# stecrotti/MatrixProductBP.jl

Measured on AMD Instinct MI355X. Metric: edge-message updates/sec (and s/sweep), SIS 3-regular N=1024 T=50 d=20, higher is better.
Workload: dtype f64

## Files before the change

### matrixproductbp.jl_amd/csrc/wg_blocks.h

```cpp
#if !defined(WG_THREADS) || !defined(WG_WAVES)
#error "define WG_THREADS / WG_WAVES and include wg_common.h before wg_blocks.h (see kernels.h)"
#endif

namespace wg {

using namespace wgc;

constexpr int GM_MB = 96;
constexpr int GM_NT = 128;
constexpr int GM_KC = 32;
constexpr int GM_LDA = 112;
constexpr int GM_LDB = 144;
constexpr int GM_LDS_DOUBLES = GM_KC * (GM_LDA + GM_LDB);

template <bool NTX = false, bool NTO = false, class SP, class XP, class OP, class SRO, class SCO, class XRO, class XCO,
          class ORO, class OCO>
__device__ __attribute__((noinline)) void gemm_direct(int M, int N, int K, SP Sp, SRO sro, SCO sco,
                                                     XP Xp, XRO xro, XCO xco, OP Op, ORO oro, OCO oco,
                                                     bool accumulate, int tile0 = -1, int tstride = WG_WAVES);

template <class SRO, class SCO, class XRO, class XCO, class ORO, class OCO>
__device__ __attribute__((noinline)) void gemm(int M, int N, int K, const gdbl* Sp, SRO sro, SCO sco, const gdbl* Xp, XRO xro,
                     XCO xco, bool xkfast, gdbl* Op, ORO oro, OCO oco, bool accumulate, ldbl* lds) {
#if WG_THREADS != 512
// ... 526 lines not shown
    const int r = j0 + tid + WG_THREADS * s;
    rv[s] = r < rows;
#pragma unroll
    for (int c = 0; c < QR_NB; c++) P[s][c] = (rv[s] && c < nb) ? Y[(long)(j0 + c) * ld + r] : 0.0;
  }
  ldbl* tot = bc;
  ldbl* rowb = bc + 32;
  qr_panel_steps<0>(P, rv, Y, ld, j0, nb, red, tau, tot, rowb);
  __syncthreads();
}

template <bool TWO>
__device__ __forceinline__ void qr_gram(const gdbl* Y, long ld, int rows32, int jrow, int jx, int nbx, int jy,
                                        int nby, int jz, int nbz, ldbl* big) {
  const int tid = threadIdx.x, lane = tid & 63, wave = __builtin_amdgcn_readfirstlane(tid >> 6);
  const int g = lane >> 4, l15 = lane & 15;
  const int nrb = (rows32 - jrow) >> 4;
  const gdbl* xcol = Y + (long)(jx + l15) * ld + jrow + 4 * g;
  const gdbl* ycol = Y + (long)(jy + l15) * ld + jrow + 4 * g;
  const gdbl* zcol = Y + (long)(jz + l15) * ld + jrow + 4 * g;
  d4 acc1 = d4{0, 0, 0, 0}, acc2 = d4{0, 0, 0, 0};
  auto head = [&](d4& v, int rb, int jv, int nbv) {
#pragma unroll
    for (int e = 0; e < 4; e++) {
      const int rr = jrow + 16 * rb + 4 * g + e - jv;
      double a = v[e];
      a = (rr < 16) ? ((rr > l15) ? a : ((rr == l15) ? 1.0 : 0.0)) : a;
      v[e] = (l15 < nbv && rr >= 0 && rb < nrb) ? a : 0.0;
    }
  };
  d4 vx[2], vy[2], vz[2];
  auto load = [&](int rb, d4& a, d4& b, d4& c) {
    const int rbc = min(rb, nrb - 1);
    a = *reinterpret_cast<const gd4*>(xcol + 16 * rbc);
    b = *reinterpret_cast<const gd4*>(ycol + 16 * rbc);
    if (TWO) c = *reinterpret_cast<const gd4*>(zcol + 16 * rbc);
  };
  auto comp = [&](int rb, d4& a, d4& b, d4& c) {
    head(a, rb, jx, nbx); head(b, rb, jy, nby);
    if (TWO) head(c, rb, jz, nbz);
#pragma unroll
    for (int e = 0; e < 4; e++) {
      acc1 = mfma(a[e], b[e], acc1);
      if (TWO) acc2 = mfma(a[e], c[e], acc2);
    }
  };
  if (wave < nrb) load(wave, vx[0], vy[0], vz[0]);
  for (int rb = wave; rb < nrb; rb += 2 * WG_WAVES) {
    load(rb + WG_WAVES, vx[1], vy[1], vz[1]);
    comp(rb, vx[0], vy[0], vz[0]);
    load(rb + 2 * WG_WAVES, vx[0], vy[0], vz[0]);
    comp(rb + WG_WAVES, vx[1], vy[1], vz[1]);
  }
#pragma unroll
  for (int r = 0; r < 4; r++) {
    big[wave * 512 + (g + 4 * r) + 16 * l15] = acc1[r];
    if (TWO) big[wave * 512 + 256 + (g + 4 * r) + 16 * l15] = acc2[r];
  }
  __syncthreads();
  if (WG_WAVES > 1) {
    constexpr int NVAL = TWO ? 512 : 256;
    constexpr int PER = (NVAL + WG_THREADS - 1) / WG_THREADS;
    double s1[PER];
#pragma unroll
    for (int e = 0; e < PER; e++) {
      const int idx = tid + e * WG_THREADS;
      s1[e] = 0.0;
      if (idx < NVAL) {
#pragma unroll
        for (int w = 0; w < WG_WAVES; w++) s1[e] += big[w * 512 + idx];
      }
    }
    __syncthreads();
#pragma unroll
    for (int e = 0; e < PER; e++) {
      const int idx = tid + e * WG_THREADS;
      if (idx < NVAL) big[idx] = s1[e];
    }
    __syncthreads();
  }
}

template <int NP>
__device__ __forceinline__ void qr_gramN(const gdbl* Y, long ld, int rows32, int jrow, int jx, const int (&jy)[NP],
                                         ldbl* big) {
  const int tid = threadIdx.x, lane = tid & 63, wave = __builtin_amdgcn_readfirstlane(tid >> 6);
  const int g = lane >> 4, l15 = lane & 15;
  const int nrb = (rows32 - jrow) >> 4;
  const gdbl* xcol = Y + (long)(jx + l15) * ld + jrow + 4 * g;
  const gdbl* ycol[NP];
  d4 acc[NP];
#pragma unroll
  for (int k = 0; k < NP; k++) { ycol[k] = Y + (long)(jy[k] + l15) * ld + jrow + 4 * g; acc[k] = d4{0, 0, 0, 0}; }
  auto head = [&](d4& v, int rb, int jv) {
#pragma unroll
    for (int e = 0; e < 4; e++) {
      const int rr = jrow + 16 * rb + 4 * g + e - jv;
      double a = v[e];
      a = (rr < 16) ? ((rr > l15) ? a : ((rr == l15) ? 1.0 : 0.0)) : a;
      v[e] = (rr >= 0 && rb < nrb) ? a : 0.0;
    }
  };
  d4 vx[2], vy[2][NP];
  auto load = [&](int rb, d4& a, d4 (&b)[NP]) {
    const int rbc = min(rb, nrb - 1);
    a = *reinterpret_cast<const gd4*>(xcol + 16 * rbc);
#pragma unroll
    for (int k = 0; k < NP; k++) b[k] = *reinterpret_cast<const gd4*>(ycol[k] + 16 * rbc);
  };
  auto comp = [&](int rb, d4& a, d4 (&b)[NP]) {
    head(a, rb, jx);
#pragma unroll
    for (int k = 0; k < NP; k++) {
      head(b[k], rb, jy[k]);
#pragma unroll
      for (int e = 0; e < 4; e++) acc[k] = mfma(a[e], b[k][e], acc[k]);
    }
  };
  if (wave < nrb) load(wave, vx[0], vy[0]);
  for (int rb = wave; rb < nrb; rb += 2 * WG_WAVES) {
    load(rb + WG_WAVES, vx[1], vy[1]);
    comp(rb, vx[0], vy[0]);
    load(rb + 2 * WG_WAVES, vx[0], vy[0]);
    comp(rb + WG_WAVES, vx[1], vy[1]);
  }
  constexpr int NVAL = 256 * NP;
#pragma unroll
  for (int k = 0; k < NP; k++)
#pragma unroll
    for (int r = 0; r < 4; r++) big[wave * NVAL + 256 * k + (g + 4 * r) + 16 * l15] = acc[k][r];
  __syncthreads();
  if (WG_WAVES > 1) {
    constexpr int PER = (NVAL + WG_THREADS - 1) / WG_THREADS;
    double s1[PER];
#pragma unroll
    for (int e = 0; e < PER; e++) {
      const int idx = tid + e * WG_THREADS;
      s1[e] = 0.0;
      if (idx < NVAL) {
#pragma unroll
        for (int w2 = 0; w2 < WG_WAVES; w2++) s1[e] += big[w2 * NVAL + idx];
      }
    }
    __syncthreads();
#pragma unroll
    for (int e = 0; e < PER; e++) {
      const int idx = tid + e * WG_THREADS;
      if (idx < NVAL) big[idx] = s1[e];
    }
    __syncthreads();
  }
}

__device__ __forceinline__ void qr_T_from_gram(const ldbl* big, const ldbl* tau, int nb, ldbl* Ts) {
  const int tid = threadIdx.x;
  if (tid < 16) {
    double trow[16];
#pragma unroll
    for (int j = 0; j < 16; j++) {
      double gcol[16];
#pragma unroll
      for (int i2 = 0; i2 < 16; i2++) gcol[i2] = big[i2 + 16 * j];
      const double tj = tau[j];
      double sacc = 0.0;
#pragma unroll
      for (int i2 = 0; i2 < j; i2++) sacc += (i2 >= tid) ? trow[i2] * gcol[i2] : 0.0;
      double v = (j == tid) ? tj : ((j > tid) ? -tj * sacc : 0.0);
      trow[j] = (j < nb) ? v : 0.0;
    }
#pragma unroll
    for (int j = 0; j < 16; j++) Ts[tid + 16 * j] = trow[j];
  }
  __syncthreads();
}

__device__ __attribute__((noinline)) void qr_panel_global(gdbl* Y, long ld, int rows, int j0, int nb, ldbl* red, ldbl* Ts,
                                       ldbl* tau, ldbl* bc) {
  const int tid = threadIdx.x, lane = tid & 63, wave = __builtin_amdgcn_readfirstlane(tid >> 6);
  for (int jj = 0; jj < nb; jj++) {
    const int col = j0 + jj;
    gdbl* x = Y + (long)col * ld;
    double ss = 0.0;
    for (int r = col + 1 + tid; r < rows; r += WG_THREADS) { double v = x[r]; ss += v * v; }
    ss = wg_sum(ss, red);
    const double alpha = x[col];
    double beta, tj, scale;
    if (ss == 0.0) { beta = alpha; tj = 0.0; scale = 0.0; }
    else {
      beta = -copysign(sqrt(alpha * alpha + ss), alpha);
      tj = (beta - alpha) / beta;
      scale = 1.0 / (alpha - beta);
    }
    __syncthreads();
    for (int r = col + 1 + tid; r < rows; r += WG_THREADS) x[r] *= scale;
    if (tid == 0) { x[col] = beta; tau[jj] = tj; }
    __syncthreads();
    double part[QR_NB];
#pragma unroll
    for (int c = 0; c < QR_NB; c++) part[c] = 0.0;
    for (int r = col + 1 + tid; r < rows; r += WG_THREADS) {
      const double v = x[r];
#pragma unroll
      for (int c = 0; c < QR_NB; c++)
        if (c != jj && c < nb) part[c] += v * Y[(long)(j0 + c) * ld + r];
    }
#pragma unroll
    for (int c = 0; c < QR_NB; c++) part[c] = wave_sum(part[c]);
    if (lane == 0) {
#pragma unroll
      for (int c = 0; c < QR_NB; c++) red[wave * 16 + c] = part[c];
    }
    __syncthreads();
    if (tid < 16) {
      double s = 0.0;
#pragma unroll
      for (int w = 0; w < WG_WAVES; w++) s += red[w * 16 + tid];
      if (tid < nb && tid != jj) s += Y[(long)(j0 + tid) * ld + col];
      bc[tid] = s;
    }
    __syncthreads();
    for (int r = col + 1 + tid; r < rows; r += WG_THREADS) {
      const double v = x[r];
      for (int c = jj + 1; c < nb; c++) Y[(long)(j0 + c) * ld + r] -= tj * bc[c] * v;
    }
    if (tid > jj && tid < nb) Y[(long)(j0 + tid) * ld + col] -= tj * bc[tid];
    if (tid < jj) {
      double s = 0.0;
      for (int i2 = tid; i2 < jj; i2++) s += Ts[tid + 16 * i2] * bc[i2];
      Ts[tid + 16 * jj] = -tj * s;
    }
    if (tid == 0) Ts[jj + 16 * jj] = tj;
    __syncthreads();
  }
}

template <int NT>
__device__ __forceinline__ void qr_trail(gdbl* Y, long ld, int rows32, int j0, int nb, int cb0, const ldbl* Ts) {
  const int lane = threadIdx.x & 63;
  const int g = lane >> 4, l15 = lane & 15;
  const int nrb = (rows32 - j0) >> 4;
  const gdbl* vcol = Y + (long)(j0 + l15) * ld + j0 + 4 * g;
  const gdbl* ccol[NT];
  d4 w0[NT];
#pragma unroll
  for (int q = 0; q < NT; q++) { ccol[q] = Y + (long)(cb0 + 16 * q + l15) * ld + j0 + 4 * g; w0[q] = d4{0, 0, 0, 0}; }
  const bool vkeep = l15 < nb;
  {
    d4 sv[3], sc[3][NT];
    auto loadA = [&](int rb, d4& v, d4 (&c)[NT]) {
      const int rbc = min(rb, nrb - 1);
      v = *reinterpret_cast<const gd4*>(vcol + 16 * rbc);
#pragma unroll
      for (int q = 0; q < NT; q++) c[q] = *reinterpret_cast<const gd4*>(ccol[q] + 16 * rbc);
      const bool keep = vkeep && rb < nrb;
#pragma unroll
      for (int e = 0; e < 4; e++) {
        const int rho = 4 * g + e;
        double x = v[e];
        x = (rb == 0) ? ((rho > l15) ? x : ((rho == l15) ? 1.0 : 0.0)) : x;
        v[e] = keep ? x : 0.0;
      }
    };
    auto compA = [&](const d4& v, const d4 (&c)[NT]) {
#pragma unroll
      for (int e = 0; e < 4; e++)
#pragma unroll
        for (int q = 0; q < NT; q++) w0[q] = mfma(v[e], c[q][e], w0[q]);
    };
    loadA(0, sv[0], sc[0]);
    loadA(1, sv[1], sc[1]);
    for (int rb = 0; rb < nrb; rb += 3) {
      loadA(rb + 2, sv[2], sc[2]); compA(sv[0], sc[0]);
      loadA(rb + 3, sv[0], sc[0]); compA(sv[1], sc[1]);
      loadA(rb + 4, sv[1], sc[1]); compA(sv[2], sc[2]);
    }
  }
  d4 w[NT];
#pragma unroll
  for (int q = 0; q < NT; q++) {
    w[q] = d4{0, 0, 0, 0};
#pragma unroll
    for (int s = 0; s < 4; s++) w[q] = mfma(Ts[(4 * s + g) + 16 * l15], w0[q][s], w[q]);
  }
  {
    const int jb = j0 & ~31;
    const int nst = (rows32 - jb) >> 5;
    for (int st = 0; st < nst; st++) {
      const int row = jb + 32 * st + 2 * l15;
      d2 v[4];
#pragma unroll
      for (int s2 = 0; s2 < 4; s2++) {
        const int k = 4 * s2 + g;
        d2 x = *reinterpret_cast<const gd2*>(Y + (long)(j0 + k) * ld + row);
#pragma unroll
        for (int e = 0; e < 2; e++) {
          const int rho = row + e - j0;
          double xe = x[e];
          xe = (rho < 16) ? ((rho > k) ? xe : ((rho == k) ? 1.0 : 0.0)) : xe;
          x[e] = (k < nb && rho >= 0) ? xe : 0.0;
        }
        v[s2] = x;
      }
      d2 c[NT][4];
#pragma unroll
      for (int q = 0; q < NT; q++)
#pragma unroll
        for (int r = 0; r < 4; r++)
          c[q][r] = *reinterpret_cast<const gd2*>(Y + (long)(cb0 + 16 * q + g + 4 * r) * ld + row);
#pragma unroll
      for (int q = 0; q < NT; q++) {
#pragma unroll
        for (int e = 0; e < 2; e++) {
          d4 acc = d4{c[q][0][e], c[q][1][e], c[q][2][e], c[q][3][e]};
#pragma unroll
          for (int s2 = 0; s2 < 4; s2++) acc = mfma_na(w[q][s2], v[s2][e], acc);
#pragma unroll
          for (int r = 0; r < 4; r++) c[q][r][e] = acc[r];
        }
#pragma unroll
        for (int r = 0; r < 4; r++)
          *reinterpret_cast<gd2*>(Y + (long)(cb0 + 16 * q + g + 4 * r) * ld + row) = c[q][r];
      }
    }
  }
}

template <int NT>
__device__ __forceinline__ void qr_trail2(gdbl* Y, long ld, int rows32, int j0, int nbb, int cb0,
                                          const ldbl* TsA, const ldbl* TsB, const ldbl* Sm) {
  const int lane = threadIdx.x & 63;
  const int g = lane >> 4, l15 = lane & 15;
  const int nrb = (rows32 - j0) >> 4;
  const gdbl* vacol = Y + (long)(j0 + l15) * ld + j0 + 4 * g;
  const gdbl* vbcol = Y + (long)(j0 + 16 + l15) * ld + j0 + 4 * g;
  const gdbl* ccol[NT];
  d4 wa0[NT], wb0[NT];
#pragma unroll
  for (int q = 0; q < NT; q++) {
    ccol[q] = Y + (long)(cb0 + 16 * q + l15) * ld + j0 + 4 * g;
    wa0[q] = d4{0, 0, 0, 0}; wb0[q] = d4{0, 0, 0, 0};
  }
  const bool bkeep = l15 < nbb;
  {
    d4 sa[3], sb[3], sc[3][NT];
    auto loadA = [&](int rb, d4& va, d4& vb, d4 (&c)[NT]) {
      const int rbc = min(rb, nrb - 1);
      va = *reinterpret_cast<const gd4*>(vacol + 16 * rbc);
      vb = *reinterpret_cast<const gd4*>(vbcol + 16 * rbc);
#pragma unroll
      for (int q = 0; q < NT; q++) c[q] = *reinterpret_cast<const gd4*>(ccol[q] + 16 * rbc);
      const bool in = rb < nrb;
#pragma unroll
      for (int e = 0; e < 4; e++) {
        const int rho = 4 * g + e;
        double a = va[e], b = vb[e];
        a = (rb == 0) ? ((rho > l15) ? a : ((rho == l15) ? 1.0 : 0.0)) : a;
        b = (rb == 1) ? ((rho > l15) ? b : ((rho == l15) ? 1.0 : 0.0)) : b;
        va[e] = in ? a : 0.0;
        vb[e] = (in && bkeep && rb >= 1) ? b : 0.0;
      }
    };
    auto compA = [&](const d4& va, const d4& vb, const d4 (&c)[NT]) {
#pragma unroll
      for (int e = 0; e < 4; e++)
#pragma unroll
        for (int q = 0; q < NT; q++) { wa0[q] = mfma(va[e], c[q][e], wa0[q]); wb0[q] = mfma(vb[e], c[q][e], wb0[q]); }
    };
    loadA(0, sa[0], sb[0], sc[0]);
    loadA(1, sa[1], sb[1], sc[1]);
    for (int rb = 0; rb < nrb; rb += 3) {
      loadA(rb + 2, sa[2], sb[2], sc[2]); compA(sa[0], sb[0], sc[0]);
      loadA(rb + 3, sa[0], sb[0], sc[0]); compA(sa[1], sb[1], sc[1]);
      loadA(rb + 4, sa[1], sb[1], sc[1]); compA(sa[2], sb[2], sc[2]);
    }
  }
  d4 wa[NT], wb[NT];
#pragma unroll
  for (int q = 0; q < NT; q++) {
    wa[q] = d4{0, 0, 0, 0};
#pragma unroll
    for (int s = 0; s < 4; s++) wa[q] = mfma(TsA[(4 * s + g) + 16 * l15], wa0[q][s], wa[q]);
    d4 t = wb0[q];
#pragma unroll
    for (int s = 0; s < 4; s++) t = mfma_na(Sm[l15 + 16 * (4 * s + g)], wa[q][s], t);
    wb[q] = d4{0, 0, 0, 0};
#pragma unroll
    for (int s = 0; s < 4; s++) wb[q] = mfma(TsB[(4 * s + g) + 16 * l15], t[s], wb[q]);
  }
  {
    const int jb = j0 & ~31;
    const int nst = (rows32 - jb) >> 5;
    for (int st = 0; st < nst; st++) {
      const int row = jb + 32 * st + 2 * l15;
      d2 va[4], vb[4];
#pragma unroll
      for (int s2 = 0; s2 < 4; s2++) {
        const int k = 4 * s2 + g;
        d2 xa = *reinterpret_cast<const gd2*>(Y + (long)(j0 + k) * ld + row);
        d2 xb = *reinterpret_cast<const gd2*>(Y + (long)(j0 + 16 + k) * ld + row);
#pragma unroll
        for (int e = 0; e < 2; e++) {
          const int ra = row + e - j0, rbb = row + e - j0 - 16;
          double a = xa[e], b = xb[e];
          a = (ra < 16) ? ((ra > k) ? a : ((ra == k) ? 1.0 : 0.0)) : a;
          b = (rbb < 16) ? ((rbb > k) ? b : ((rbb == k) ? 1.0 : 0.0)) : b;
          xa[e] = (ra >= 0) ? a : 0.0;
          xb[e] = (k < nbb && rbb >= 0) ? b : 0.0;
        }
        va[s2] = xa; vb[s2] = xb;
      }
      d2 c[NT][4];
#pragma unroll
      for (int q = 0; q < NT; q++)
#pragma unroll
        for (int r = 0; r < 4; r++)
          c[q][r] = *reinterpret_cast<const gd2*>(Y + (long)(cb0 + 16 * q + g + 4 * r) * ld + row);
#pragma unroll
      for (int q = 0; q < NT; q++) {
#pragma unroll
        for (int e = 0; e < 2; e++) {
          d4 acc = d4{c[q][0][e], c[q][1][e], c[q][2][e], c[q][3][e]};
#pragma unroll
          for (int s2 = 0; s2 < 4; s2++) { acc = mfma_na(wa[q][s2], va[s2][e], acc); acc = mfma_na(wb[q][s2], vb[s2][e], acc); }
#pragma unroll
          for (int r = 0; r < 4; r++) c[q][r][e] = acc[r];
        }
#pragma unroll
        for (int r = 0; r < 4; r++)
          *reinterpret_cast<gd2*>(Y + (long)(cb0 + 16 * q + g + 4 * r) * ld + row) = c[q][r];
      }
    }
  }
}

__device__ __forceinline__ void qr_tile_update_all(gdbl* Y, long ld, int rows32, int j0, int nb, int cb0,
                                                   const ldbl* Ts, ldbl* big) {
  const int tid = threadIdx.x, lane = tid & 63, wave = __builtin_amdgcn_readfirstlane(tid >> 6);
  const int g = lane >> 4, l15 = lane & 15;
  const int nrb = (rows32 - j0) >> 4;
  const gdbl* vcol = Y + (long)(j0 + l15) * ld + j0 + 4 * g;
  const gdbl* ccol = Y + (long)(cb0 + l15) * ld + j0 + 4 * g;
  d4 acc = d4{0, 0, 0, 0};
  for (int rb = wave; rb < nrb; rb += WG_WAVES) {
    d4 v = *reinterpret_cast<const gd4*>(vcol + 16 * rb);
    d4 c = *reinterpret_cast<const gd4*>(ccol + 16 * rb);
#pragma unroll
    for (int e = 0; e < 4; e++) {
      const int rho = 4 * g + e;
      double x = v[e];
      x = (rb == 0) ? ((rho > l15) ? x : ((rho == l15) ? 1.0 : 0.0)) : x;
      v[e] = (l15 < nb) ? x : 0.0;
    }
#pragma unroll
    for (int e = 0; e < 4; e++) acc = mfma(v[e], c[e], acc);
  }
#pragma unroll
  for (int r = 0; r < 4; r++) big[wave * 256 + (g + 4 * r) + 16 * l15] = acc[r];
  __syncthreads();
  d4 w0 = d4{0, 0, 0, 0};
#pragma unroll
  for (int w = 0; w < WG_WAVES; w++)
#pragma unroll
    for (int r = 0; r < 4; r++) w0[r] += big[w * 256 + (g + 4 * r) + 16 * l15];
  d4 wv = d4{0, 0, 0, 0};
#pragma unroll
  for (int s = 0; s < 4; s++) wv = mfma(Ts[(4 * s + g) + 16 * l15], w0[s], wv);
  const int jb = j0 & ~31;
  const int nst = (rows32 - jb) >> 5;
  for (int st = wave; st < nst; st += WG_WAVES) {
    const int row = jb + 32 * st + 2 * l15;
    d2 v[4], c[4];
#pragma unroll
    for (int s2 = 0; s2 < 4; s2++) {
      const int k = 4 * s2 + g;
      d2 x = *reinterpret_cast<const gd2*>(Y + (long)(j0 + k) * ld + row);
#pragma unroll
      for (int e = 0; e < 2; e++) {
        const int rho = row + e - j0;
        double xe = x[e];
        xe = (rho < 16) ? ((rho > k) ? xe : ((rho == k) ? 1.0 : 0.0)) : xe;
        x[e] = (k < nb && rho >= 0) ? xe : 0.0;
      }
      v[s2] = x;
    }
#pragma unroll
    for (int r = 0; r < 4; r++) c[r] = *reinterpret_cast<const gd2*>(Y + (long)(cb0 + g + 4 * r) * ld + row);
#pragma unroll
    for (int e = 0; e < 2; e++) {
      d4 a = d4{c[0][e], c[1][e], c[2][e], c[3][e]};
#pragma unroll
      for (int s2 = 0; s2 < 4; s2++) a = mfma_na(wv[s2], v[s2][e], a);
#pragma unroll
      for (int r = 0; r < 4; r++) c[r][e] = a[r];
    }
#pragma unroll
    for (int r = 0; r < 4; r++) *reinterpret_cast<gd2*>(Y + (long)(cb0 + g + 4 * r) * ld + row) = c[r];
  }
  __syncthreads();
}

template <int NT>
__device__ __forceinline__ void qr_tile_update2_all(gdbl* Y, long ld, int rows32, int j0, int cb0, const ldbl* TsA,
                                                    const ldbl* TsB, const ldbl* Sm, ldbl* big) {
  const int tid = threadIdx.x, lane = tid & 63, wave = __builtin_amdgcn_readfirstlane(tid >> 6);
  const int g = lane >> 4, l15 = lane & 15;
  const int nrb = (rows32 - j0) >> 4;
  const gdbl* vacol = Y + (long)(j0 + l15) * ld + j0 + 4 * g;
  const gdbl* vbcol = Y + (long)(j0 + 16 + l15) * ld + j0 + 4 * g;
  d4 acca[NT], accb[NT];
#pragma unroll
  for (int q = 0; q < NT; q++) { acca[q] = d4{0, 0, 0, 0}; accb[q] = d4{0, 0, 0, 0}; }
  for (int rb = wave; rb < nrb; rb += WG_WAVES) {
    d4 va = *reinterpret_cast<const gd4*>(vacol + 16 * rb);
    d4 vb = *reinterpret_cast<const gd4*>(vbcol + 16 * rb);
    d4 c[NT];
#pragma unroll
    for (int q = 0; q < NT; q++) c[q] = *reinterpret_cast<const gd4*>(Y + (long)(cb0 + 16 * q + l15) * ld + j0 + 4 * g + 16 * rb);
#pragma unroll
    for (int e = 0; e < 4; e++) {
      const int rho = 4 * g + e;
      double a = va[e], b = vb[e];
      a = (rb == 0) ? ((rho > l15) ? a : ((rho == l15) ? 1.0 : 0.0)) : a;
      b = (rb == 1) ? ((rho > l15) ? b : ((rho == l15) ? 1.0 : 0.0)) : b;
      va[e] = a;
      vb[e] = (rb >= 1) ? b : 0.0;
    }
#pragma unroll
    for (int e = 0; e < 4; e++)
#pragma unroll
      for (int q = 0; q < NT; q++) { acca[q] = mfma(va[e], c[q][e], acca[q]); accb[q] = mfma(vb[e], c[q][e], accb[q]); }
  }
  constexpr int NVAL = 512 * NT;
#pragma unroll
  for (int q = 0; q < NT; q++)
#pragma unroll
    for (int r = 0; r < 4; r++) {
      big[wave * NVAL + 512 * q + (g + 4 * r) + 16 * l15] = acca[q][r];
      big[wave * NVAL + 512 * q + 256 + (g + 4 * r) + 16 * l15] = accb[q][r];
    }
  __syncthreads();
  d4 wa[NT], wb[NT];
#pragma unroll
  for (int q = 0; q < NT; q++) {
    d4 wa0 = d4{0, 0, 0, 0}, wb0 = d4{0, 0, 0, 0};
#pragma unroll
    for (int w = 0; w < WG_WAVES; w++)
#pragma unroll
      for (int r = 0; r < 4; r++) {
        wa0[r] += big[w * NVAL + 512 * q + (g + 4 * r) + 16 * l15];
        wb0[r] += big[w * NVAL + 512 * q + 256 + (g + 4 * r) + 16 * l15];
      }
    wa[q] = d4{0, 0, 0, 0}; wb[q] = d4{0, 0, 0, 0};
#pragma unroll
    for (int s = 0; s < 4; s++) wa[q] = mfma(TsA[(4 * s + g) + 16 * l15], wa0[s], wa[q]);
    d4 t = wb0;
#pragma unroll
    for (int s = 0; s < 4; s++) t = mfma_na(Sm[l15 + 16 * (4 * s + g)], wa[q][s], t);
#pragma unroll
    for (int s = 0; s < 4; s++) wb[q] = mfma(TsB[(4 * s + g) + 16 * l15], t[s], wb[q]);
  }
  const int jb = j0 & ~31;
  const int nst = (rows32 - jb) >> 5;
  for (int st = wave; st < nst; st += WG_WAVES) {
    const int row = jb + 32 * st + 2 * l15;
    d2 va[4], vb[4];
#pragma unroll
    for (int s2 = 0; s2 < 4; s2++) {
      const int k = 4 * s2 + g;
      d2 xa = *reinterpret_cast<const gd2*>(Y + (long)(j0 + k) * ld + row);
      d2 xb = *reinterpret_cast<const gd2*>(Y + (long)(j0 + 16 + k) * ld + row);
#pragma unroll
      for (int e = 0; e < 2; e++) {
        const int ra = row + e - j0, rbb = row + e - j0 - 16;
        double a = xa[e], b = xb[e];
        a = (ra < 16) ? ((ra > k) ? a : ((ra == k) ? 1.0 : 0.0)) : a;
        b = (rbb < 16) ? ((rbb > k) ? b : ((rbb == k) ? 1.0 : 0.0)) : b;
        xa[e] = (ra >= 0) ? a : 0.0;
        xb[e] = (rbb >= 0) ? b : 0.0;
      }
      va[s2] = xa; vb[s2] = xb;
    }
#pragma unroll
    for (int q = 0; q < NT; q++) {
      d2 c[4];
#pragma unroll
      for (int r = 0; r < 4; r++) c[r] = *reinterpret_cast<const gd2*>(Y + (long)(cb0 + 16 * q + g + 4 * r) * ld + row);
#pragma unroll
      for (int e = 0; e < 2; e++) {
        d4 acc = d4{c[0][e], c[1][e], c[2][e], c[3][e]};
#pragma unroll
        for (int s2 = 0; s2 < 4; s2++) { acc = mfma_na(wa[q][s2], va[s2][e], acc); acc = mfma_na(wb[q][s2], vb[s2][e], acc); }
#pragma unroll
        for (int r = 0; r < 4; r++) c[r][e] = acc[r];
      }
#pragma unroll
      for (int r = 0; r < 4; r++) *reinterpret_cast<gd2*>(Y + (long)(cb0 + 16 * q + g + 4 * r) * ld + row) = c[r];
    }
  }
  __syncthreads();
}

template <int NT>
__device__ __forceinline__ void qr_trail4(gdbl* Y, long ld, int rows32, int j0, int cb0, const ldbl* const (&Tq)[4],
                                          const ldbl* const (&Sq)[6]) {
  const int lane = threadIdx.x & 63;
  const int g = lane >> 4, l15 = lane & 15;
  const int nrb = (rows32 - j0) >> 4;
  const gdbl* vcol[4];
#pragma unroll
  for (int p = 0; p < 4; p++) vcol[p] = Y + (long)(j0 + 16 * p + l15) * ld + j0 + 4 * g;
  const gdbl* ccol[NT];
  d4 w0[4][NT];
#pragma unroll
  for (int q = 0; q < NT; q++) {
    ccol[q] = Y + (long)(cb0 + 16 * q + l15) * ld + j0 + 4 * g;
#pragma unroll
    for (int p = 0; p < 4; p++) w0[p][q] = d4{0, 0, 0, 0};
  }
  {
    d4 sv[2][4], sc[2][NT];
    auto loadA = [&](int rb, d4 (&v)[4], d4 (&c)[NT]) {
      const int rbc = min(rb, nrb - 1);
#pragma unroll
      for (int p = 0; p < 4; p++) v[p] = *reinterpret_cast<const gd4*>(vcol[p] + 16 * rbc);
#pragma unroll
      for (int q = 0; q < NT; q++) c[q] = __builtin_nontemporal_load(reinterpret_cast<const gd4*>(ccol[q] + 16 * rbc));
      const bool in = rb < nrb;
#pragma unroll
      for (int p = 0; p < 4; p++)
#pragma unroll
        for (int e = 0; e < 4; e++) {
          const int rho = 4 * g + e;
          double a = v[p][e];
          a = (rb == p) ? ((rho > l15) ? a : ((rho == l15) ? 1.0 : 0.0)) : a;
          v[p][e] = (in && rb >= p) ? a : 0.0;
        }
    };
    auto compA = [&](const d4 (&v)[4], const d4 (&c)[NT]) {
#pragma unroll
      for (int e = 0; e < 4; e++)
#pragma unroll
        for (int q = 0; q < NT; q++)
#pragma unroll
          for (int p = 0; p < 4; p++) w0[p][q] = mfma(v[p][e], c[q][e], w0[p][q]);
    };
    loadA(0, sv[0], sc[0]);
    for (int rb = 0; rb < nrb; rb += 2) {
      loadA(rb + 1, sv[1], sc[1]); compA(sv[0], sc[0]);
      loadA(rb + 2, sv[0], sc[0]); compA(sv[1], sc[1]);
    }
  }
  d4 w[4][NT];
#pragma unroll
  for (int q = 0; q < NT; q++) {
#pragma unroll
    for (int p = 0; p < 4; p++) {
      d4 t = w0[p][q];
#pragma unroll
      for (int r = 0; r < p; r++) {
        const ldbl* S = Sq[p * (p - 1) / 2 + r];
#pragma unroll
        for (int s = 0; s < 4; s++) t = mfma_na(S[l15 + 16 * (4 * s + g)], w[r][q][s], t);
      }
      d4 o = d4{0, 0, 0, 0};
#pragma unroll
      for (int s = 0; s < 4; s++) o = mfma(Tq[p][(4 * s + g) + 16 * l15], t[s], o);
      w[p][q] = o;
    }
  }
  {
    const int jb = j0 & ~31;
    const int nst = (rows32 - jb) >> 5;
    for (int st = 0; st < nst; st++) {
      const int row = jb + 32 * st + 2 * l15;
      d2 v[4][4];
#pragma unroll
      for (int p = 0; p < 4; p++)
#pragma unroll
        for (int s2 = 0; s2 < 4; s2++) {
          const int k = 4 * s2 + g;
          d2 x = *reinterpret_cast<const gd2*>(Y + (long)(j0 + 16 * p + k) * ld + row);
#pragma unroll
          for (int e = 0; e < 2; e++) {
            const int rp = row + e - j0 - 16 * p;
            double a = x[e];
            a = (rp < 16) ? ((rp > k) ? a : ((rp == k) ? 1.0 : 0.0)) : a;
            x[e] = (rp >= 0) ? a : 0.0;
          }
          v[p][s2] = x;
        }
      d2 c[NT][4];
#pragma unroll
      for (int q = 0; q < NT; q++)
#pragma unroll
        for (int r = 0; r < 4; r++)
          c[q][r] = __builtin_nontemporal_load(reinterpret_cast<const gd2*>(Y + (long)(cb0 + 16 * q + g + 4 * r) * ld + row));
#pragma unroll
      for (int q = 0; q < NT; q++) {
#pragma unroll
        for (int e = 0; e < 2; e++) {
          d4 acc = d4{c[q][0][e], c[q][1][e], c[q][2][e], c[q][3][e]};
#pragma unroll
          for (int s2 = 0; s2 < 4; s2++)
#pragma unroll
// ... 185 lines not shown
              const d2 va = *reinterpret_cast<const ld2*>(vp), vbb = *reinterpret_cast<const ld2*>(vp + 2);
              const double v4[4] = {va[0], va[1], vbb[0], vbb[1]};
#pragma unroll
              for (int e = 0; e < 4; e++)
#pragma unroll
                for (int q = 0; q < NR; q++) w0[p][q] = mfma(v4[e], cc[q][rb][e], w0[p][q]);
            }
          }
#pragma unroll
          for (int q = 0; q < NR; q++) { cc[q][0] = cn[q][0]; cc[q][1] = cn[q][1]; }
        }
        stage_store(m + 1, h, vn);
      }
    }
  }
  d4 w[4][NR];
  if (NTL > 0) {
#pragma unroll
    for (int q = 0; q < NR; q++) {
#pragma unroll
      for (int p = 0; p < 4; p++) {
        d4 t = w0[p][q];
#pragma unroll
        for (int r = 0; r < p; r++) {
          const ldbl* S = Sq[p * (p - 1) / 2 + r];
#pragma unroll
          for (int s = 0; s < 4; s++) t = mfma_na(S[l15 + 16 * (4 * s + g)], w[r][q][s], t);
        }
        d4 o = d4{0, 0, 0, 0};
#pragma unroll
        for (int s = 0; s < 4; s++) o = mfma(Tq[p][(4 * s + g) + 16 * l15], t[s], o);
        w[p][q] = o;
      }
    }
  }
  {
    {
      const d4 v0 = stage_load(0, 0), v1 = stage_load(0, 1);
      __syncthreads();
      stage_store(0, 0, v0); stage_store(0, 1, v1);
    }
    gdbl* cp[NR];
#pragma unroll
    for (int q = 0; q < NR; q++) cp[q] = Y + (long)(cq[q] + g) * ld + j0 + 2 * l15;
    d2 cc[NR][4];
    if (NTL > 0) {
#pragma unroll
      for (int q = 0; q < NR; q++)
#pragma unroll
        for (int r = 0; r < 4; r++) cc[q][r] = __builtin_nontemporal_load(reinterpret_cast<const gd2*>(cp[q] + (long)(4 * r) * ld));
    }
    for (int m = 0; m < nms; m++) {
#pragma unroll 1
      for (int h = 0; h < 2; h++) {
        const d4 vn = stage_load(m + 1, h);
        const int s = 2 * m + h;
        const int sn = min(s + 1, nst - 1);
        d2 cn[NR][4];
        if (NTL > 0) {
#pragma unroll
          for (int q = 0; q < NR; q++)
#pragma unroll
            for (int r = 0; r < 4; r++)
              cn[q][r] = __builtin_nontemporal_load(reinterpret_cast<const gd2*>(cp[q] + (long)(4 * r) * ld + 32 * sn));
        }
        if (h == 0) lds_barrier();
        if (NTL > 0) {
          if (s < nst) {
            const ldbl* vb = Vs + (m & 1) * QR_VM_STAGE + 32 * h;
            d4 acc[NR][2];
#pragma unroll
            for (int q = 0; q < NR; q++)
#pragma unroll
              for (int e = 0; e < 2; e++) acc[q][e] = d4{cc[q][0][e], cc[q][1][e], cc[q][2][e], cc[q][3][e]};
#pragma unroll
            for (int p = 0; p < 4; p++)
#pragma unroll
              for (int s2 = 0; s2 < 4; s2++) {
                const d2 v = *reinterpret_cast<const ld2*>(vb + (16 * p + 4 * s2 + g) * QR_VM_LD + 2 * l15);
#pragma unroll
                for (int e = 0; e < 2; e++)
#pragma unroll
                  for (int q = 0; q < NR; q++) acc[q][e] = mfma_na(w[p][q][s2], v[e], acc[q][e]);
              }
#pragma unroll
            for (int q = 0; q < NR; q++)
#pragma unroll
              for (int r = 0; r < 4; r++)
                __builtin_nontemporal_store(d2{acc[q][0][r], acc[q][1][r]}, reinterpret_cast<gd2*>(cp[q] + (long)(4 * r) * ld + 32 * s));
          }
#pragma unroll
          for (int q = 0; q < NR; q++)
#pragma unroll
            for (int r = 0; r < 4; r++) cc[q][r] = cn[q][r];
        }
        stage_store(m + 1, h, vn);
      }
    }
  }
}

__device__ __attribute__((noinline)) void qr_trail4_coop(gdbl* Y, long ld, int rows32, int j0, int cstart, int ntl,
                                                         const ldbl* const (&Tq)[4], const ldbl* const (&Sq)[6], ldbl* Vs) {
  const int wave = __builtin_amdgcn_readfirstlane(threadIdx.x >> 6);
  const int nst = (rows32 - j0) >> 5;
  const int tbase = ntl / WG_WAVES, trem = ntl % WG_WAVES;
  const int tcnt = tbase + (wave < trem ? 1 : 0);
  const int tstart = wave * tbase + min(wave, trem);
  const int npass = (tbase + (trem ? 1 : 0) + 1) >> 1;
  for (int pass = 0; pass < npass; pass++) {
    const int t0 = 2 * pass;
    const int nt = __builtin_amdgcn_readfirstlane(max(0, min(2, tcnt - t0)));
    const int cb0 = cstart + 16 * (tstart + t0);
    if (nt == 2) qr_trail4_coop_pass<2>(Y, ld, j0, nst, cb0, cb0 + 16, Tq, Sq, Vs);
    else if (nt == 1) qr_trail4_coop_pass<1>(Y, ld, j0, nst, cb0, cb0, Tq, Sq, Vs);
    else qr_trail4_coop_pass<0>(Y, ld, j0, nst, cstart, cstart, Tq, Sq, Vs);
  }
  __syncthreads();
}

__device__ __attribute__((noinline)) void qr_r(gdbl* Y, long ld, int rows, int cols, ldbl* lds, ldbl* big, Prof* pr = nullptr,
                     unsigned long long* plast = nullptr, int ph_panel = 0, int ph_trail = 0, bool force_generic = false) {
  const int tid = threadIdx.x, lane = tid & 63, wave = __builtin_amdgcn_readfirstlane(tid >> 6);
  const int g = lane >> 4, l15 = lane & 15;
  ldbl* red = lds;
  ldbl* Ts = lds + 2 * WG_WAVES * 16;
  ldbl* tau = Ts + 256;
  ldbl* bc = tau + 16;
  const int kmax = min(rows, cols);
  const bool fine = pr && ph_panel < 0;
  const int rows16 = (rows + 15) & ~15;
  const int rows32 = (rows + 31) & ~31;

  ldbl* TsB = lds + QR_LDS_BASE;
  ldbl* Sm = TsB + 256;
  ldbl* tauB = Sm + 256;
  ldbl* TsC = lds + QR_LDS_PAIR;
  ldbl* TsD = TsC + 256;
  ldbl* Sdc = TsD + 256;
  ldbl* Sca = Sdc + 256;
  ldbl* Scb = Sca + 256;
  ldbl* Sda = Scb + 256;
  ldbl* Sdb = Sda + 256;
  ldbl* tauC = Sdb + 256;
  ldbl* tauD = tauC + 16;

  auto factor_panel = [&](int jp, int nbp, ldbl* Tp, ldbl* taup) {
    for (int i = tid; i < 256; i += WG_THREADS) Tp[i] = 0.0;
    if (tid < 16) taup[tid] = 0.0;
    __syncthreads();
    qr_panel_regs(Y, ld, rows, jp, nbp, red, taup, bc);
    if (fine) prof_mark(pr, *plast, 14);
  };
  auto factor_pair = [&](int jp, ldbl* T1, ldbl* tau1, ldbl* T2, ldbl* tau2, ldbl* S21) {
    factor_panel(jp, 16, T1, tau1);
    qr_gram<false>(Y, ld, rows32, jp, jp, 16, jp, 16, jp, 16, big);
    if (fine) prof_mark(pr, *plast, 15);
    qr_T_from_gram(big, tau1, 16, T1);
    if (pr) prof_mark(pr, *plast, fine ? 16 : ph_panel);
    qr_tile_update_all(Y, ld, rows32, jp, 16, jp + 16, T1, big);
    if (pr) prof_mark(pr, *plast, fine ? 17 : ph_trail);
    factor_panel(jp + 16, 16, T2, tau2);
    qr_gram<true>(Y, ld, rows32, jp, jp + 16, 16, jp + 16, 16, jp, 16, big);
    for (int i = tid; i < 256; i += WG_THREADS) S21[i] = big[256 + i];
    if (fine) prof_mark(pr, *plast, 15);
    qr_T_from_gram(big, tau2, 16, T2);
    if (pr) prof_mark(pr, *plast, fine ? 16 : ph_panel);
  };
  auto factor_pair2 = [&](int ja) {
    const int jc = ja + 32, jd = ja + 48;
    factor_panel(jc, 16, TsC, tauC);
    { const int jy[3] = {jc, ja, ja + 16}; qr_gramN<3>(Y, ld, rows32, jc, jc, jy, big); }
    for (int i = tid; i < 256; i += WG_THREADS) { Sca[i] = big[256 + i]; Scb[i] = big[512 + i]; }
    if (fine) prof_mark(pr, *plast, 15);
    qr_T_from_gram(big, tauC, 16, TsC);
    if (pr) prof_mark(pr, *plast, fine ? 16 : ph_panel);
    qr_tile_update_all(Y, ld, rows32, jc, 16, jd, TsC, big);
    if (pr) prof_mark(pr, *plast, fine ? 17 : ph_trail);
    factor_panel(jd, 16, TsD, tauD);
    { const int jy[4] = {jd, jc, ja, ja + 16}; qr_gramN<4>(Y, ld, rows32, jd, jd, jy, big); }
    for (int i = tid; i < 256; i += WG_THREADS) { Sdc[i] = big[256 + i]; Sda[i] = big[512 + i]; Sdb[i] = big[768 + i]; }
    if (fine) prof_mark(pr, *plast, 15);
    qr_T_from_gram(big, tauD, 16, TsD);
    if (pr) prof_mark(pr, *plast, fine ? 16 : ph_panel);
  };
  auto wave_tiles = [&](int cstart, int& tstart, int& tcnt) {
    const int ntl = (cols - cstart + 15) / 16;
    const int tbase = ntl / WG_WAVES, trem = ntl % WG_WAVES;
    tcnt = tbase + (wave < trem ? 1 : 0);
    tstart = wave * tbase + min(wave, trem);
  };

  for (int j0 = 0; j0 < kmax;) {
    const int nb = min(QR_NB, kmax - j0);
    const bool fast = !force_generic && rows - j0 <= QR_RS * WG_THREADS;
    const bool quad = QR_QUAD && fast && j0 + 64 <= kmax && j0 + 64 < cols;
    const bool pair = !quad && fast && j0 + 32 <= kmax && j0 + 32 < cols;
    if (quad) {
      factor_pair(j0, Ts, tau, TsB, tauB, Sm);
      qr_tile_update2_all<2>(Y, ld, rows32, j0, j0 + 32, Ts, TsB, Sm, big);
      if (pr) prof_mark(pr, *plast, fine ? 17 : ph_trail);
      factor_pair2(j0);
      const ldbl* const Tq[4] = {Ts, TsB, TsC, TsD};
      const ldbl* const Sq[6] = {Sm, Sca, Scb, Sda, Sdb, Sdc};
      const int ntl4 = (cols - (j0 + 64) + 15) / 16;
      if (WG_WAVES > 1 && ntl4 <= QR_ROWPAR_TILES) {
        for (int tl = 0; tl < ntl4; tl++) qr_tile_update4_all(Y, ld, rows32, j0, j0 + 64 + 16 * tl, Tq, Sq, big);
      } else if (WG_WAVES == 8 && !QR_TRAIL_PER_WAVE) {
        const int rem = ((ntl4 & 3) == 1 && ntl4 > 4) ? 1 : 0;
        qr_trail4_coop(Y, ld, rows32, j0, j0 + 64, ntl4 - rem, Tq, Sq, big);
        if (rem) qr_tile_update4_all(Y, ld, rows32, j0, j0 + 64 + 16 * (ntl4 - 1), Tq, Sq, big);
      } else {
        int tstart, tcnt;
        wave_tiles(j0 + 64, tstart, tcnt);
        for (int tg = 0; tg < tcnt; tg += 2) {
          const int cb0 = j0 + 64 + (tstart + tg) * 16;
          if (tcnt - tg >= 2) qr_trail4<2>(Y, ld, rows32, j0, cb0, Tq, Sq);
          else qr_trail4<1>(Y, ld, rows32, j0, cb0, Tq, Sq);
        }
      }
      __syncthreads();
      if (pr) prof_mark(pr, *plast, fine ? 18 : ph_trail);
      j0 += 64;
      continue;
    }
    if (pair) factor_pair(j0, Ts, tau, TsB, tauB, Sm);
    else {
      for (int i = tid; i < 256; i += WG_THREADS) Ts[i] = 0.0;
      if (tid < 16) tau[tid] = 0.0;
      __syncthreads();
      if (fast) {
        qr_panel_regs(Y, ld, rows, j0, nb, red, tau, bc);
        if (fine) prof_mark(pr, *plast, 14);
        qr_gram<false>(Y, ld, rows32, j0, j0, nb, j0, nb, j0, nb, big);
        if (fine) prof_mark(pr, *plast, 15);
        qr_T_from_gram(big, tau, nb, Ts);
      } else qr_panel_global(Y, ld, rows, j0, nb, red, Ts, tau, bc);
      if (pr) prof_mark(pr, *plast, fine ? 16 : ph_panel);
    }
    const int cstart = pair ? j0 + 32 : j0 + nb;
    int tstart, tcnt;
    wave_tiles(cstart, tstart, tcnt);
    for (int tg = 0; tg < tcnt; tg += QR_TC) {
      const int nt = min(QR_TC, tcnt - tg);
      const int cb0 = cstart + (tstart + tg) * 16;
      if (pair) {
        if (nt == 1) qr_trail2<1>(Y, ld, rows32, j0, 16, cb0, Ts, TsB, Sm);
        else if (nt == 2) qr_trail2<2>(Y, ld, rows32, j0, 16, cb0, Ts, TsB, Sm);
        else qr_trail2<3>(Y, ld, rows32, j0, 16, cb0, Ts, TsB, Sm);
      } else {
        if (nt == 1) qr_trail<1>(Y, ld, rows32, j0, nb, cb0, Ts);
        else if (nt == 2) qr_trail<2>(Y, ld, rows32, j0, nb, cb0, Ts);
        else qr_trail<3>(Y, ld, rows32, j0, nb, cb0, Ts);
      }
    }
    __syncthreads();
    if (pr) prof_mark(pr, *plast, fine ? 18 : ph_trail);
    j0 += pair ? 32 : 16;
  }
  (void)g; (void)l15; (void)lane;
}

__device__ __forceinline__ void jac_cs(double al, double be, double ga, double& c, double& s) {
  const double d = be - al, g2 = 2.0 * ga;
  const double h2 = d * d + g2 * g2;
  double rs = __builtin_amdgcn_rsq(h2);
  rs = rs * (1.5 - 0.5 * h2 * rs * rs);
  double hy = h2 * rs;
  hy = hy + 0.5 * rs * (h2 - hy * hy);
  const double den = fabs(d) + hy;
  double rd = __builtin_amdgcn_rcp(den);
  rd = rd * (2.0 - den * rd);
  rd = rd * (2.0 - den * rd);
  const double t = copysign(g2, d * ga) * rd;
  const double o2 = 1.0 + t * t;
  c = __builtin_amdgcn_rsq(o2);
  c = c * (1.5 - 0.5 * o2 * c * c);
  c = c * (1.5 - 0.5 * o2 * c * c);
  s = c * t;
}

template <int R, class AP>
__device__ __forceinline__ double jac_pair8(AP ap, AP aq, int sub, double tol, double nul) {
  double x[R], y[R];
#pragma unroll
  for (int i = 0; i < R; i++) { x[i] = ap[sub + 8 * i]; y[i] = aq[sub + 8 * i]; }
  double al = 0, be = 0, ga = 0;
#pragma unroll
  for (int i = 0; i < R; i++) { al += x[i] * x[i]; be += y[i] * y[i]; ga += x[i] * y[i]; }
  al += dpp64<0x141>(al); be += dpp64<0x141>(be); ga += dpp64<0x141>(ga);
  al += dpp64<0x4E>(al); be += dpp64<0x4E>(be); ga += dpp64<0x4E>(ga);
  al += dpp64<0xB1>(al); be += dpp64<0xB1>(be); ga += dpp64<0xB1>(ga);
  if (!(ga * ga > (tol * tol) * (al * be) && al > nul && be > nul)) return 0.0;
  double c, s;
  jac_cs(al, be, ga, c, s);
#pragma unroll
  for (int i = 0; i < R; i++) { ap[sub + 8 * i] = c * x[i] - s * y[i]; aq[sub + 8 * i] = s * x[i] + c * y[i]; }
  return ga * ga / (al * be);
}

template <class T> struct jac_in_hbm { static constexpr bool value = false; };
template <> struct jac_in_hbm<gdbl*> { static constexpr bool value = true; };

__device__ __forceinline__ double jac_pair_hbm16(gdbl* ap, gdbl* aq, int sub, int m, double tol, double nul) {
  typedef double d2_t __attribute__((ext_vector_type(2)));
  typedef __attribute__((address_space(1))) d2_t gd2_t;
  constexpr int JP = 6;
  const int npl = (m + 15) >> 4;
  double al = 0, be = 0, ga = 0;
  d2_t x[JP], y[JP];
  auto loadc = [&](int j0) {
#pragma unroll
    for (int j = 0; j < JP; j++) {
      const int r = 2 * (sub + 8 * (j0 + j));
      const bool ok0 = r < m, ok1 = r + 1 < m;
      const int rc = ok1 ? r : 2 * sub;
      const d2_t xv = *reinterpret_cast<const gd2_t*>(ap + rc), yv = *reinterpret_cast<const gd2_t*>(aq + rc);
      x[j] = d2_t{ok0 && ok1 ? xv[0] : 0.0, ok1 ? xv[1] : 0.0};
      y[j] = d2_t{ok0 && ok1 ? yv[0] : 0.0, ok1 ? yv[1] : 0.0};
    }
  };
  for (int j0 = 0; j0 < npl; j0 += JP) {
    loadc(j0);
#pragma unroll
    for (int j = 0; j < JP; j++) {
      al += x[j][0] * x[j][0]; be += y[j][0] * y[j][0]; ga += x[j][0] * y[j][0];
      al += x[j][1] * x[j][1]; be += y[j][1] * y[j][1]; ga += x[j][1] * y[j][1];
    }
  }
  al += dpp64<0x141>(al); be += dpp64<0x141>(be); ga += dpp64<0x141>(ga);
  al += dpp64<0x4E>(al); be += dpp64<0x4E>(be); ga += dpp64<0x4E>(ga);
  al += dpp64<0xB1>(al); be += dpp64<0xB1>(be); ga += dpp64<0xB1>(ga);
  if (!(ga * ga > (tol * tol) * (al * be) && al > nul && be > nul)) return 0.0;
  double c, s;
  jac_cs(al, be, ga, c, s);
  for (int j0 = 0; j0 < npl; j0 += JP) {
    if (npl > JP) loadc(j0);
#pragma unroll
    for (int j = 0; j < JP; j++) {
      const int r = 2 * (sub + 8 * (j0 + j));
      if (r + 1 < m) {
        *reinterpret_cast<gd2_t*>(ap + r) = d2_t{c * x[j][0] - s * y[j][0], c * x[j][1] - s * y[j][1]};
        *reinterpret_cast<gd2_t*>(aq + r) = d2_t{s * x[j][0] + c * y[j][0], s * x[j][1] + c * y[j][1]};
      }
    }
  }
  return ga * ga / (al * be);
}

template <class AP>
__device__ __attribute__((noinline)) int jacobi_rsv(AP A, int lda, int m, int n, double* V, int ldv, ldbl* red,
                                                    __attribute__((address_space(3))) int* act, int maxsweeps) {
  const int tid = threadIdx.x;
  if (V) {
    for (int idx = tid; idx < n * n; idx += WG_THREADS) {
      int r = idx % n, c = idx / n;
      V[r + (long)ldv * c] = (r == c) ? 1.0 : 0.0;
    }
  }
  for (int c = tid; c < n; c += WG_THREADS) act[c] = c;
  __syncthreads();
  if (n < 2) return 0;
  double fro2 = 0.0;
  for (int idx = tid; idx < m * n; idx += WG_THREADS) { double v = A[(idx % m) + (long)lda * (idx / m)]; fro2 += v * v; }
  fro2 = wg_sum(fro2, red);
  const double nul = 1e-28 * fro2;
  const double tol = 1e-15;
  constexpr int JC = 12;
  int nact = n;
  int sweep = 0;
  bool conv = false;
  for (; sweep < maxsweeps; sweep++) {
    const int ne = (nact + 1) & ~1;
    const int npairs = ne / 2;
    int lg = 3;
    while (lg > 0 && (npairs << lg) > WG_THREADS) lg--;
    while (lg < 3 && ((m + (1 << lg) - 1) >> lg) > JC) lg++;
    const int LP = 1 << lg;
    const int sub = tid & (LP - 1);
// ... 106 lines not shown
```

Before: 547.8.

## Fuse QR trailing-update W0 products into multi-panel Gram reductions

```diff
diff --git a/matrixproductbp.jl_amd/csrc/wg_blocks.h b/matrixproductbp.jl_amd/csrc/wg_blocks.h
--- a/matrixproductbp.jl_amd/csrc/wg_blocks.h
+++ b/matrixproductbp.jl_amd/csrc/wg_blocks.h
@@ -702,6 +702,81 @@
   }
 }
 
+template <int NP, int NPR>
+__device__ __forceinline__ void qr_gram_multi(const gdbl* Y, long ld, int rows32, int jrow, const int (&jc)[NP],
+                                              const bool (&hd)[NP], const int (&pa)[NPR], const int (&pb)[NPR], ldbl* big) {
+  const int tid = threadIdx.x, lane = tid & 63, wave = __builtin_amdgcn_readfirstlane(tid >> 6);
+  const int g = lane >> 4, l15 = lane & 15;
+  const int nrb = (rows32 - jrow) >> 4;
+  const gdbl* col[NP];
+#pragma unroll
+  for (int p = 0; p < NP; p++) col[p] = Y + (long)(jc[p] + l15) * ld + jrow + 4 * g;
+  d4 acc[NPR];
+#pragma unroll
+  for (int k = 0; k < NPR; k++) acc[k] = d4{0, 0, 0, 0};
+  auto mask = [&](d4& v, int rb, int p) {
+#pragma unroll
+    for (int e = 0; e < 4; e++) {
+      const int rr = jrow + 16 * rb + 4 * g + e - jc[p];
+      double a = v[e];
+      if (hd[p]) a = (rr < 16) ? ((rr > l15) ? a : ((rr == l15) ? 1.0 : 0.0)) : a;
+      v[e] = (rb < nrb) ? a : 0.0;
+    }
+  };
+  d4 x[2][NP];
+  auto load = [&](int rb, d4 (&b)[NP]) {
+    const int rbc = min(rb, nrb - 1);
+#pragma unroll
+    for (int p = 0; p < NP; p++) b[p] = *reinterpret_cast<const gd4*>(col[p] + 16 * rbc);
+  };
+  auto comp = [&](int rb, d4 (&b)[NP]) {
+#pragma unroll
+    for (int p = 0; p < NP; p++) mask(b[p], rb, p);
+#pragma unroll
+    for (int k = 0; k < NPR; k++)
+#pragma unroll
+      for (int e = 0; e < 4; e++) acc[k] = mfma(b[pa[k]][e], b[pb[k]][e], acc[k]);
+  };
+  if (wave < nrb) load(wave, x[0]);
+  for (int rb = wave; rb < nrb; rb += 2 * WG_WAVES) {
+    load(rb + WG_WAVES, x[1]);
+    comp(rb, x[0]);
+    load(rb + 2 * WG_WAVES, x[0]);
+    comp(rb + WG_WAVES, x[1]);
+  }
+  constexpr int NR = (NPR + 3) / 4;
+  constexpr int PER = (1024 + WG_THREADS - 1) / WG_THREADS;
+  double s1[NR][PER];
+#pragma unroll
+  for (int rd = 0; rd < NR; rd++) {
+    const int nk = min(4, NPR - 4 * rd);
+    if (rd > 0) __syncthreads();
+#pragma unroll
+    for (int k = 4 * rd; k < min(4 * rd + 4, NPR); k++)
+#pragma unroll
+      for (int r = 0; r < 4; r++) big[wave * 1024 + 256 * (k - 4 * rd) + (g + 4 * r) + 16 * l15] = acc[k][r];
+    __syncthreads();
+#pragma unroll
+    for (int e = 0; e < PER; e++) {
+      const int idx = tid + e * WG_THREADS;
+      s1[rd][e] = 0.0;
+      if (idx < 256 * nk) {
+#pragma unroll
+        for (int w = 0; w < WG_WAVES; w++) s1[rd][e] += big[w * 1024 + idx];
+      }
+    }
+  }
+  __syncthreads();
+#pragma unroll
+  for (int rd = 0; rd < NR; rd++)
+#pragma unroll
+    for (int e = 0; e < PER; e++) {
+      const int idx = tid + e * WG_THREADS;
+      if (idx < 256 * min(4, NPR - 4 * rd)) big[1024 * rd + idx] = s1[rd][e];
+    }
+  __syncthreads();
+}
+
 __device__ __forceinline__ void qr_T_from_gram(const ldbl* big, const ldbl* tau, int nb, ldbl* Ts) {
   const int tid = threadIdx.x;
   if (tid < 16) {
@@ -984,14 +1059,14 @@
 }
 
 __device__ __forceinline__ void qr_tile_update_all(gdbl* Y, long ld, int rows32, int j0, int nb, int cb0,
-                                                   const ldbl* Ts, ldbl* big) {
+                                                   const ldbl* Ts, ldbl* big, const ldbl* W0f = nullptr) {
   const int tid = threadIdx.x, lane = tid & 63, wave = __builtin_amdgcn_readfirstlane(tid >> 6);
   const int g = lane >> 4, l15 = lane & 15;
   const int nrb = (rows32 - j0) >> 4;
   const gdbl* vcol = Y + (long)(j0 + l15) * ld + j0 + 4 * g;
   const gdbl* ccol = Y + (long)(cb0 + l15) * ld + j0 + 4 * g;
   d4 acc = d4{0, 0, 0, 0};
-  for (int rb = wave; rb < nrb; rb += WG_WAVES) {
+  for (int rb = W0f ? nrb : wave; rb < nrb; rb += WG_WAVES) {
     d4 v = *reinterpret_cast<const gd4*>(vcol + 16 * rb);
     d4 c = *reinterpret_cast<const gd4*>(ccol + 16 * rb);
 #pragma unroll
@@ -1004,14 +1079,19 @@
 #pragma unroll
     for (int e = 0; e < 4; e++) acc = mfma(v[e], c[e], acc);
   }
-#pragma unroll
-  for (int r = 0; r < 4; r++) big[wave * 256 + (g + 4 * r) + 16 * l15] = acc[r];
-  __syncthreads();
   d4 w0 = d4{0, 0, 0, 0};
-#pragma unroll
-  for (int w = 0; w < WG_WAVES; w++)
-#pragma unroll
-    for (int r = 0; r < 4; r++) w0[r] += big[w * 256 + (g + 4 * r) + 16 * l15];
+  if (W0f) {
+#pragma unroll
+    for (int r = 0; r < 4; r++) w0[r] = W0f[(g + 4 * r) + 16 * l15];
+  } else {
+#pragma unroll
+    for (int r = 0; r < 4; r++) big[wave * 256 + (g + 4 * r) + 16 * l15] = acc[r];
+    __syncthreads();
+#pragma unroll
+    for (int w = 0; w < WG_WAVES; w++)
+#pragma unroll
+      for (int r = 0; r < 4; r++) w0[r] += big[w * 256 + (g + 4 * r) + 16 * l15];
+  }
   d4 wv = d4{0, 0, 0, 0};
 #pragma unroll
   for (int s = 0; s < 4; s++) wv = mfma(Ts[(4 * s + g) + 16 * l15], w0[s], wv);
@@ -1051,55 +1131,19 @@
 
 template <int NT>
 __device__ __forceinline__ void qr_tile_update2_all(gdbl* Y, long ld, int rows32, int j0, int cb0, const ldbl* TsA,
-                                                    const ldbl* TsB, const ldbl* Sm, ldbl* big) {
+                                                    const ldbl* TsB, const ldbl* Sm, const ldbl* W0) {
   const int tid = threadIdx.x, lane = tid & 63, wave = __builtin_amdgcn_readfirstlane(tid >> 6);
   const int g = lane >> 4, l15 = lane & 15;
-  const int nrb = (rows32 - j0) >> 4;
-  const gdbl* vacol = Y + (long)(j0 + l15) * ld + j0 + 4 * g;
-  const gdbl* vbcol = Y + (long)(j0 + 16 + l15) * ld + j0 + 4 * g;
-  d4 acca[NT], accb[NT];
-#pragma unroll
-  for (int q = 0; q < NT; q++) { acca[q] = d4{0, 0, 0, 0}; accb[q] = d4{0, 0, 0, 0}; }
-  for (int rb = wave; rb < nrb; rb += WG_WAVES) {
-    d4 va = *reinterpret_cast<const gd4*>(vacol + 16 * rb);
-    d4 vb = *reinterpret_cast<const gd4*>(vbcol + 16 * rb);
-    d4 c[NT];
-#pragma unroll
-    for (int q = 0; q < NT; q++) c[q] = *reinterpret_cast<const gd4*>(Y + (long)(cb0 + 16 * q + l15) * ld + j0 + 4 * g + 16 * rb);
-#pragma unroll
-    for (int e = 0; e < 4; e++) {
-      const int rho = 4 * g + e;
-      double a = va[e], b = vb[e];
-      a = (rb == 0) ? ((rho > l15) ? a : ((rho == l15) ? 1.0 : 0.0)) : a;
-      b = (rb == 1) ? ((rho > l15) ? b : ((rho == l15) ? 1.0 : 0.0)) : b;
-      va[e] = a;
-      vb[e] = (rb >= 1) ? b : 0.0;
-    }
-#pragma unroll
-    for (int e = 0; e < 4; e++)
-#pragma unroll
-      for (int q = 0; q < NT; q++) { acca[q] = mfma(va[e], c[q][e], acca[q]); accb[q] = mfma(vb[e], c[q][e], accb[q]); }
-  }
-  constexpr int NVAL = 512 * NT;
-#pragma unroll
-  for (int q = 0; q < NT; q++)
+  (void)tid;
+  d4 wa[NT], wb[NT];
+#pragma unroll
+  for (int q = 0; q < NT; q++) {
+    d4 wa0, wb0;
 #pragma unroll
     for (int r = 0; r < 4; r++) {
-      big[wave * NVAL + 512 * q + (g + 4 * r) + 16 * l15] = acca[q][r];
-      big[wave * NVAL + 512 * q + 256 + (g + 4 * r) + 16 * l15] = accb[q][r];
-    }
-  __syncthreads();
-  d4 wa[NT], wb[NT];
-#pragma unroll
-  for (int q = 0; q < NT; q++) {
-    d4 wa0 = d4{0, 0, 0, 0}, wb0 = d4{0, 0, 0, 0};
-#pragma unroll
-    for (int w = 0; w < WG_WAVES; w++)
-#pragma unroll
-      for (int r = 0; r < 4; r++) {
-        wa0[r] += big[w * NVAL + 512 * q + (g + 4 * r) + 16 * l15];
-        wb0[r] += big[w * NVAL + 512 * q + 256 + (g + 4 * r) + 16 * l15];
-      }
+      wa0[r] = W0[512 * q + (g + 4 * r) + 16 * l15];
+      wb0[r] = W0[512 * q + 256 + (g + 4 * r) + 16 * l15];
+    }
     wa[q] = d4{0, 0, 0, 0}; wb[q] = d4{0, 0, 0, 0};
 #pragma unroll
     for (int s = 0; s < 4; s++) wa[q] = mfma(TsA[(4 * s + g) + 16 * l15], wa0[s], wa[q]);
@@ -1591,16 +1635,24 @@
     qr_panel_regs(Y, ld, rows, jp, nbp, red, taup, bc);
     if (fine) prof_mark(pr, *plast, 14);
   };
-  auto factor_pair = [&](int jp, ldbl* T1, ldbl* tau1, ldbl* T2, ldbl* tau2, ldbl* S21) {
+  auto factor_pair = [&](int jp, ldbl* T1, ldbl* tau1, ldbl* T2, ldbl* tau2, ldbl* S21, bool quad4) {
     factor_panel(jp, 16, T1, tau1);
-    qr_gram<false>(Y, ld, rows32, jp, jp, 16, jp, 16, jp, 16, big);
+    if (QR_QUAD) {
+      const int jc[2] = {jp, jp + 16}; const bool hd[2] = {true, false};
+      const int pa[2] = {0, 0}, pb[2] = {0, 1};
+      qr_gram_multi<2, 2>(Y, ld, rows32, jp, jc, hd, pa, pb, big);
+    } else qr_gram<false>(Y, ld, rows32, jp, jp, 16, jp, 16, jp, 16, big);
     if (fine) prof_mark(pr, *plast, 15);
     qr_T_from_gram(big, tau1, 16, T1);
     if (pr) prof_mark(pr, *plast, fine ? 16 : ph_panel);
-    qr_tile_update_all(Y, ld, rows32, jp, 16, jp + 16, T1, big);
+    qr_tile_update_all(Y, ld, rows32, jp, 16, jp + 16, T1, big, QR_QUAD ? big + 256 : nullptr);
     if (pr) prof_mark(pr, *plast, fine ? 17 : ph_trail);
     factor_panel(jp + 16, 16, T2, tau2);
-    qr_gram<true>(Y, ld, rows32, jp, jp + 16, 16, jp + 16, 16, jp, 16, big);
+    if (QR_QUAD && quad4) {
+      const int jc[4] = {jp + 16, jp, jp + 32, jp + 48}; const bool hd[4] = {true, true, false, false};
+      const int pa[6] = {0, 0, 1, 0, 1, 0}, pb[6] = {0, 1, 2, 2, 3, 3};
+      qr_gram_multi<4, 6>(Y, ld, rows32, jp, jc, hd, pa, pb, big);
+    } else qr_gram<true>(Y, ld, rows32, jp, jp + 16, 16, jp + 16, 16, jp, 16, big);
     for (int i = tid; i < 256; i += WG_THREADS) S21[i] = big[256 + i];
     if (fine) prof_mark(pr, *plast, 15);
     qr_T_from_gram(big, tau2, 16, T2);
@@ -1609,12 +1661,16 @@
   auto factor_pair2 = [&](int ja) {
     const int jc = ja + 32, jd = ja + 48;
     factor_panel(jc, 16, TsC, tauC);
-    { const int jy[3] = {jc, ja, ja + 16}; qr_gramN<3>(Y, ld, rows32, jc, jc, jy, big); }
+    {
+      const int jq[4] = {jc, ja, ja + 16, jd}; const bool hd[4] = {true, true, true, false};
+      const int pa[4] = {0, 0, 0, 0}, pb[4] = {0, 1, 2, 3};
+      qr_gram_multi<4, 4>(Y, ld, rows32, jc, jq, hd, pa, pb, big);
+    }
     for (int i = tid; i < 256; i += WG_THREADS) { Sca[i] = big[256 + i]; Scb[i] = big[512 + i]; }
     if (fine) prof_mark(pr, *plast, 15);
     qr_T_from_gram(big, tauC, 16, TsC);
     if (pr) prof_mark(pr, *plast, fine ? 16 : ph_panel);
-    qr_tile_update_all(Y, ld, rows32, jc, 16, jd, TsC, big);
+    qr_tile_update_all(Y, ld, rows32, jc, 16, jd, TsC, big, big + 768);
     if (pr) prof_mark(pr, *plast, fine ? 17 : ph_trail);
     factor_panel(jd, 16, TsD, tauD);
     { const int jy[4] = {jd, jc, ja, ja + 16}; qr_gramN<4>(Y, ld, rows32, jd, jd, jy, big); }
@@ -1636,8 +1692,8 @@
     const bool quad = QR_QUAD && fast && j0 + 64 <= kmax && j0 + 64 < cols;
     const bool pair = !quad && fast && j0 + 32 <= kmax && j0 + 32 < cols;
     if (quad) {
-      factor_pair(j0, Ts, tau, TsB, tauB, Sm);
-      qr_tile_update2_all<2>(Y, ld, rows32, j0, j0 + 32, Ts, TsB, Sm, big);
+      factor_pair(j0, Ts, tau, TsB, tauB, Sm, true);
+      qr_tile_update2_all<2>(Y, ld, rows32, j0, j0 + 32, Ts, TsB, Sm, big + 512);
       if (pr) prof_mark(pr, *plast, fine ? 17 : ph_trail);
       factor_pair2(j0);
       const ldbl* const Tq[4] = {Ts, TsB, TsC, TsD};
@@ -1663,7 +1719,7 @@
       j0 += 64;
       continue;
     }
-    if (pair) factor_pair(j0, Ts, tau, TsB, tauB, Sm);
+    if (pair) factor_pair(j0, Ts, tau, TsB, tauB, Sm, false);
     else {
       for (int i = tid; i < 256; i += WG_THREADS) Ts[i] = 0.0;
       if (tid < 16) tau[tid] = 0.0;
```

New measurement: 572.1, median of 6. +4.4%, better.
